# OrangeSodahub/ORV

Measured on AMD Instinct MI355X. Metric: denoise-steps/sec, higher is better.
Workload: dtype bf16; 1 GPU; configs[1]: CogVideoX-2B singleview 320x480x17f (latents [B,5,32,40,60], S=3226), DDIM 50-step schedule, guidance 1.0, trajectory-conditioned; batch_per_gpu=4, num_layers=30, parallelism=replica x1 (no collective), valid=True

## Files before the change

orv_amd/csrc/norm.hip:

```cpp
#include "common.hpp"
#include "mxfp8.hpp"

namespace {

#ifndef ORV_LN_WAVES
#define ORV_LN_WAVES 1
#endif
template <int CH, bool FULL, bool MX = false>
__global__ __launch_bounds__(256, ORV_LN_WAVES) void ln_mod_kernel(const bf16_t* __restrict__ x, long ldx, bf16_t* __restrict__ y,
                                                     long ldy, const bf16_t* __restrict__ gamma,
                                                     const bf16_t* __restrict__ beta, const float* __restrict__ scale,
                                                     const float* __restrict__ shift, long mod_b, long mod_g, int seq,
                                                     int n_text, int per_group, int rows, int D, float eps,
                                                     orv_rowmap_t xmap, uint8_t* __restrict__ mxs) {
    const int lane = threadIdx.x & 63;
    const int row = blockIdx.x * 4 + (threadIdx.x >> 6);
    if (row >= rows) return;
    const int nchunk = D >> 3;
    const long xrow = xmap.rows > 0 ? (long)(row / xmap.rows) * xmap.bstride + xmap.off + row % xmap.rows : row;
    const bf16_t* xr = x + xrow * ldx;
    uint4 raw[CH];
    int ce[CH];
    bool ok[CH];
#pragma unroll
// ... 175 lines not shown
#pragma unroll
        for (int k = 0; k < 16; ++k) o[vt_pos(k)] = vt_s[grp * 16 + k][d];
        bf16_t* dst = vT + ((long)(b * H + h) * 64 + d) * s_pad + s0 + grp * 16;
        uint4 a, c2;
        a.x = o[0] | ((uint32_t)o[1] << 16); a.y = o[2] | ((uint32_t)o[3] << 16);
        a.z = o[4] | ((uint32_t)o[5] << 16); a.w = o[6] | ((uint32_t)o[7] << 16);
        c2.x = o[8] | ((uint32_t)o[9] << 16); c2.y = o[10] | ((uint32_t)o[11] << 16);
        c2.z = o[12] | ((uint32_t)o[13] << 16); c2.w = o[14] | ((uint32_t)o[15] << 16);
        *(uint4*)dst = a;
        *(uint4*)(dst + 8) = c2;
    }
}

#ifndef ORV_LNR_WAVES
#define ORV_LNR_WAVES 3
#endif
__device__ __forceinline__ uint4 lnr_load(const bf16_t* p) {
#ifdef ORV_LNR_NT_LOAD
    typedef unsigned nt_u32x4 __attribute__((ext_vector_type(4)));
    const nt_u32x4 v = __builtin_nontemporal_load((const nt_u32x4*)p);
    return make_uint4(v[0], v[1], v[2], v[3]);
#else
    return *(const uint4*)p;
#endif
}
__device__ __forceinline__ void lnr_store(bf16_t* p, const uint4 u) {
#ifdef ORV_LNR_NT_STORE
    typedef unsigned nt_u32x4 __attribute__((ext_vector_type(4)));
    __builtin_nontemporal_store(nt_u32x4{u.x, u.y, u.z, u.w}, (nt_u32x4*)p);
#else
    *(uint4*)p = u;
#endif
}
template <int CH, bool PACKED = false, bool MX = false>
__global__ __launch_bounds__(256, ORV_LNR_WAVES) void ln_mod_rows_kernel(const bf16_t* __restrict__ x, long ldx, bf16_t* __restrict__ y, long ldy,
                                                             const bf16_t* __restrict__ gamma, const bf16_t* __restrict__ beta,
                                                             const float* __restrict__ scale, const float* __restrict__ shift, long mod_b,
                                                             long mod_g, int seq, int n_text, int per_group, int rows, int D, float eps, int R,
                                                             uint8_t* __restrict__ mxs) {
    const int lane = threadIdx.x & 63;
    const int w = blockIdx.x * 4 + (threadIdx.x >> 6);
    const int r0 = __builtin_amdgcn_readfirstlane(w * R);
    if (r0 >= rows) return;
    const int r1 = min(r0 + R, rows);
    const int nchunk = D >> 3;
    int ce[CH];
    bool ok[CH];
#pragma unroll
    for (int i = 0; i < CH; ++i) {
        const int c = lane + 64 * i;
        ok[i] = c < nchunk;
        ce[i] = min(c, nchunk - 1);
    }
    float gg[CH][8], hh[CH][8];
    long cur_off = -1;
    uint4 raw[CH];
#pragma unroll
    for (int i = 0; i < CH; ++i) raw[i] = lnr_load(x + (long)r0 * ldx + ce[i] * 8);
    for (int row = r0; row < r1; ++row) {
        const int b = row / seq, sidx = row % seq;
        const long off = b * mod_b + orv_group_of(sidx, n_text, per_group) * mod_g;
        if (off != cur_off) {
            cur_off = off;
#pragma unroll
            for (int i = 0; i < CH; ++i) {
                const uint4 gm = *(const uint4*)(gamma + ce[i] * 8), bt = *(const uint4*)(beta + ce[i] * 8);
                const float4 s0 = *(const float4*)(scale + off + ce[i] * 8), s1 = *(const float4*)(scale + off + ce[i] * 8 + 4);
                const float4 h0 = *(const float4*)(shift + off + ce[i] * 8), h1 = *(const float4*)(shift + off + ce[i] * 8 + 4);
                const float sv[8] = {s0.x, s0.y, s0.z, s0.w, s1.x, s1.y, s1.z, s1.w};
                const float hv[8] = {h0.x, h0.y, h0.z, h0.w, h1.x, h1.y, h1.z, h1.w};
                const uint32_t gw[4] = {gm.x, gm.y, gm.z, gm.w}, bw[4] = {bt.x, bt.y, bt.z, bt.w};
#pragma unroll
                for (int e = 0; e < 8; ++e) {
                    const float g = bf2f((e & 1) ? gw[e >> 1] >> 16 : gw[e >> 1] & 0xffff);
                    const float be = bf2f((e & 1) ? bw[e >> 1] >> 16 : bw[e >> 1] & 0xffff);
                    gg[i][e] = g * (1.0f + sv[e]);
                    hh[i][e] = fmaf(be, 1.0f + sv[e], hv[e]);
                }
                __builtin_amdgcn_sched_barrier(0);
            }
        }
        float v[CH][8];
        float s = 0.f;
#pragma unroll
        for (int i = 0; i < CH; ++i) {
            const uint32_t wv[4] = {raw[i].x, raw[i].y, raw[i].z, raw[i].w};
#pragma unroll
            for (int e = 0; e < 4; ++e) {
                v[i][2 * e] = bf2f(wv[e] & 0xffff);
                v[i][2 * e + 1] = bf2f(wv[e] >> 16);
                s += ok[i] ? v[i][2 * e] + v[i][2 * e + 1] : 0.f;
            }
        }
        {
            const int rn = min(row + 1, rows - 1);
#pragma unroll
            for (int i = 0; i < CH; ++i) raw[i] = lnr_load(x + (long)rn * ldx + ce[i] * 8);
        }
        const float mean = wave_sum_valu(s) / (float)D;
        float sq = 0.f;
#pragma unroll
        for (int i = 0; i < CH; ++i) {
#pragma unroll
            for (int e = 0; e < 8; ++e) {
                const float d = ok[i] ? v[i][e] - mean : 0.f;
                sq += d * d;
            }
        }
        const float rstd = rsqrtf(wave_sum_valu(sq) / (float)D + eps);
        bf16_t* yr = y + (long)row * ldy;
#pragma unroll
        for (int i = 0; i < CH; ++i) {
            float o[8];
#pragma unroll
            for (int e = 0; e < 8; ++e) o[e] = fmaf((v[i][e] - mean) * rstd, gg[i][e], hh[i][e]);
            uint4 u;
            u.x = pack2bf(o[0], o[1]); u.y = pack2bf(o[2], o[3]); u.z = pack2bf(o[4], o[5]); u.w = pack2bf(o[6], o[7]);
            if constexpr (MX) {
                uint2 qq;
                uint32_t sb;
                mx_quantize8(u, qq, sb);
                if (ok[i]) mx_store8((uint8_t*)y + (long)row * ldy, mxs + (long)row * (D >> 5), ce[i], qq, sb);
            } else if (PACKED) *(uint4*)(y + ((((long)(row >> 4) * (D >> 5) + (ce[i] >> 2)) << 9) + ((((ce[i] & 3) << 4) + (row & 15)) << 3))) = u;
            else lnr_store(yr + ce[i] * 8, u);
        }
    }
}

}

static int layernorm_modulate_impl(const void* x, int ldx, orv_rowmap_t xmap, void* y, int ldy, const void* gamma,
                                   const void* beta, const float* scale, const float* shift, long mod_b, long mod_g,
                                   orv_groups_t grp, int batch, int D, float eps, void* stream, bool packed, uint8_t* mxs = nullptr) {
    ORV_REQUIRE(x && y, "orv_layernorm_modulate: null operand");
    ORV_REQUIRE(D % 8 == 0 && D <= 4096, "orv_layernorm_modulate: D=%d must be a multiple of 8 and <= 4096", D);
    ORV_REQUIRE(grp.seq > 0 && batch > 0, "orv_layernorm_modulate: empty problem");
    ORV_REQUIRE((scale == nullptr) == (shift == nullptr), "orv_layernorm_modulate: scale and shift go together");
    ORV_REQUIRE(ldx % 8 == 0 && ldy % 8 == 0, "orv_layernorm_modulate: misaligned rows");
    const int rows = batch * grp.seq;
    const int ch = (D / 8 + 63) / 64;
    dim3 grid((rows + 3) / 4), block(256);
    hipStream_t st = (hipStream_t)stream;
    const bool full = gamma && beta && scale && shift;
    const bool mx = mxs != nullptr;
    ORV_REQUIRE(!mx || (!packed && D % 32 == 0), "orv_layernorm_modulate_mxfp8: D=%d must be a multiple of 32", D);
    static int rows_env = -2;
    if (rows_env == -2) { const char* e = getenv("ORV_LN_ROWS"); rows_env = e ? atoi(e) : -1; }
    ORV_REQUIRE(!packed || (full && xmap.rows == 0 && ch <= 4 && D % 32 == 0 && ldy == D),
                "orv_layernorm_modulate_packed: needs gamma, beta, scale, shift, no row map, D %% 32 == 0, D <= 2048 and ldy == D");
    if (full && xmap.rows == 0 && (packed || rows_env != 0) && ch <= 4) {
        const int slots = 256 * 4 * ORV_LNR_WAVES;
        const int R = rows_env > 0 ? rows_env : max(rows >= 2048 ? 2 : 1, (rows + slots - 1) / slots);
        dim3 g2(((rows + R - 1) / R + 3) / 4);
#define ORV_LNR_CASE(C)                                                                                                \
        if (mx)                                                                                                        \
            hipLaunchKernelGGL((ln_mod_rows_kernel<C, false, true>), g2, block, 0, st, (const bf16_t*)x, (long)ldx, (bf16_t*)y, (long)ldy, \
                               (const bf16_t*)gamma, (const bf16_t*)beta, scale, shift, mod_b, mod_g, grp.seq, grp.n_text, \
                               grp.per_group, rows, D, eps, R, mxs);                                                   \
        else if (packed)                                                                                               \
            hipLaunchKernelGGL((ln_mod_rows_kernel<C, true>), g2, block, 0, st, (const bf16_t*)x, (long)ldx, (bf16_t*)y, (long)ldy, \
                               (const bf16_t*)gamma, (const bf16_t*)beta, scale, shift, mod_b, mod_g, grp.seq, grp.n_text, \
                               grp.per_group, rows, D, eps, R, nullptr);                                               \
// ... 60 lines not shown
                            const float* rope_cos, const float* rope_sin, int B, int S, int H, int n_text, int s_pad,
                            float eps, float q_premul, void* stream) {
    return orv_qkv_prep_from(qkv, qkv, vT, gq, bq, gk, bk, rope_cos, rope_sin, B, S, H, n_text, s_pad, eps, q_premul, stream);
}

extern "C" int orv_qkv_prep_from(const void* src, void* qkv, void* vT, const void* gq, const void* bq, const void* gk,
                                 const void* bk, const float* rope_cos, const float* rope_sin, int B, int S, int H, int n_text,
                                 int s_pad, float eps, float q_premul, void* stream) {
    ORV_REQUIRE(src && qkv, "orv_qkv_prep: null operand");
    ORV_REQUIRE(B > 0 && S > 0 && H > 0, "orv_qkv_prep: empty problem");
    ORV_REQUIRE(s_pad % 64 == 0 && s_pad >= S && s_pad == ((S + 63) / 64) * 64,
                "orv_qkv_prep: s_pad=%d must be S=%d rounded up to 64", s_pad, S);
    ORV_REQUIRE((rope_cos == nullptr) == (rope_sin == nullptr), "orv_qkv_prep: cos and sin go together");
    dim3 grid(s_pad / 64, H, B);
    hipLaunchKernelGGL(qkv_prep_kernel, grid, dim3(256), 0, (hipStream_t)stream, (const bf16_t*)src, (bf16_t*)qkv, (bf16_t*)vT,
                       (const bf16_t*)gq, (const bf16_t*)bq, (const bf16_t*)gk, (const bf16_t*)bk, rope_cos, rope_sin, S,
                       H, n_text, s_pad, eps, q_premul);
    return orv_check_launch("orv_qkv_prep");
}

namespace {

struct ModArgs {
    const bf16_t* temb;
    const bf16_t* act;
    const bf16_t* const* W;
    const bf16_t* const* bias;
    float* out;
    int n_tab, B, T, E, width, text;
    int vis_tiles;
};

template <int KS>
__device__ __forceinline__ void mod_cond_frags(const ModArgs& p, int b, int t, bool is_text, bool rvalid, int hi, bf16x8 (&cf)[KS]) {
    const bool has_act = !is_text && p.act != nullptr;
    const bf16_t* tp = p.temb + (long)b * p.E + hi * 8;
    const bf16_t* ap = has_act ? p.act + ((long)b * p.T + t) * p.E + hi * 8 : tp;
    constexpr int BATCH = KS < 8 ? KS : 8;
#pragma unroll
    for (int k0 = 0; k0 < KS; k0 += BATCH) {
        uint4 tu[BATCH], au[BATCH];
#pragma unroll
        for (int j = 0; j < BATCH; ++j) { tu[j] = *(const uint4*)(tp + (k0 + j) * 16); au[j] = *(const uint4*)(ap + (k0 + j) * 16); }
#pragma unroll
        for (int j = 0; j < BATCH; ++j) {
            const uint32_t tw[4] = {tu[j].x, tu[j].y, tu[j].z, tu[j].w}, aw[4] = {au[j].x, au[j].y, au[j].z, au[j].w};
            union { bf16x8 v; uint32_t u[4]; } c;
#pragma unroll
            for (int e = 0; e < 4; ++e) {
                float lo = bf2f(tw[e] & 0xffff), hi2 = bf2f(tw[e] >> 16);
                const float lo_a = bf2f(f2bf(lo + bf2f(aw[e] & 0xffff))), hi_a = bf2f(f2bf(hi2 + bf2f(aw[e] >> 16)));
                lo = has_act ? lo_a : lo;
                hi2 = has_act ? hi_a : hi2;
                c.u[e] = rvalid ? pack2bf(silu(lo), silu(hi2)) : 0u;
            }
            cf[k0 + j] = c.v;
        }
    }
}

template <int KS>
__global__ __launch_bounds__(256) void mod_tables_kernel(const ModArgs p) {
    const int lane = threadIdx.x & 63, wave = threadIdx.x >> 6;
    const int l31 = lane & 31, hi = lane >> 5;
    const int tab = blockIdx.y;
    const bool is_text = (int)blockIdx.z >= p.vis_tiles;
    const int rtile = is_text ? blockIdx.z - p.vis_tiles : blockIdx.z;
    const int nrows = is_text ? p.B : p.B * p.T;
    const int r = rtile * 32 + l31;
    const bool rvalid = r < nrows;
// ... 30 lines not shown
                    o.x += bf2f(bb.x & 0xffff); o.y += bf2f(bb.x >> 16); o.z += bf2f(bb.y & 0xffff); o.w += bf2f(bb.y >> 16);
                }
                *(float4*)(orow + n) = o;
            }
        }
    }
}

}

namespace {
__device__ __forceinline__ void mt_glds16(const void* gsrc, const void* lds_dst) {
    unsigned keep;
    const unsigned d = __builtin_amdgcn_readfirstlane((unsigned)(uintptr_t)(const __attribute__((address_space(3))) char*)lds_dst);
    asm volatile("s_mov_b32 %0, m0\n\ts_mov_b32 m0, %2\n\ts_nop 0\n\tglobal_load_lds_dwordx4 %1, off\n\ts_mov_b32 m0, %0"
                 : "=&s"(keep) : "v"(gsrc), "s"(d) : "memory");
}
constexpr int MT_SLABS = 4;
constexpr int MT_MAXBLK = 4;
__global__ __launch_bounds__(256) void mod_tables_lds_kernel(const ModArgs p) {
    constexpr int KS = 32, SPB = 8;
    __shared__ __attribute__((aligned(16))) char smem[4 * MT_SLABS * 4096];
    const int lane = threadIdx.x & 63, wave = __builtin_amdgcn_readfirstlane(threadIdx.x >> 6);
    const int l31 = lane & 31, hi = lane >> 5, sw = (l31 >> 1) & 7;
    const int tab = blockIdx.y;
    const bool is_text = (int)blockIdx.z >= p.vis_tiles;
    const int rtile = is_text ? blockIdx.z - p.vis_tiles : blockIdx.z;
    const int nrows = is_text ? p.B : p.B * p.T;
    const int r = rtile * 32 + l31;
    const bool rvalid = r < nrows;
    const int b = rvalid ? (is_text ? r : r / p.T) : 0;
    const int t = rvalid && !is_text ? r % p.T : 0;
    bf16x8 cf[KS];
    mod_cond_frags<KS>(p, b, t, is_text, rvalid, hi, cf);
    const bf16_t* Wt = p.W[tab] + (is_text ? (long)p.width * p.E : 0);
    const bf16_t* bt = p.bias ? (p.bias[tab] ? p.bias[tab] + (is_text ? p.width : 0) : nullptr) : nullptr;
    const int G = 1 + p.T;
    float* orow = p.out + (((long)tab * p.B + b) * G + (is_text ? 0 : 1 + t)) * p.width;
    const int nblocks = p.width / 32;
    const int nb0 = blockIdx.x * 4 + wave, stride = gridDim.x * 4;
    const int nblk = nb0 < nblocks ? (nblocks - nb0 + stride - 1) / stride : 0;
    const int total = nblk * SPB;
    char* const ring = smem + wave * (MT_SLABS * 4096);
    int soff[4];
#pragma unroll
    for (int j = 0; j < 4; ++j) {
        const int row = 8 * j + (lane >> 3);
        soff[j] = row * p.E + (((lane & 7) ^ ((row >> 1) & 7)) << 3);
    }
    auto issue = [&](int sl) {
        const int bi = sl / SPB, ks = sl % SPB;
        const bf16_t* wp = Wt + (long)((nb0 + bi * stride) * 32) * p.E + ks * 64;
        char* const d = ring + (sl % MT_SLABS) * 4096;
#pragma unroll
        for (int j = 0; j < 4; ++j) mt_glds16(wp + soff[j], d + j * 1024);
    };
    f32x16 acc[MT_MAXBLK];
#pragma unroll
    for (int i = 0; i < MT_MAXBLK; ++i)
#pragma unroll
        for (int e = 0; e < 16; ++e) acc[i][e] = 0.f;
#pragma unroll
    for (int sl = 0; sl < MT_SLABS - 1; ++sl)
        if (sl < total) issue(sl);
    const int rd_off = l31 * 128;
#pragma unroll
    for (int bi = 0; bi < MT_MAXBLK; ++bi) {
// ... 70 lines not shown
```

orv_amd/csrc/gemm_d8.hip:

```cpp
#include "gemm_common.hpp"

namespace {
using namespace orv_gemm;

__device__ __forceinline__ void d8_unpack8(const uint4 u, float (&f)[8]) {
    f[0] = bf2f(u.x & 0xffff); f[1] = bf2f(u.x >> 16); f[2] = bf2f(u.y & 0xffff); f[3] = bf2f(u.y >> 16);
    f[4] = bf2f(u.z & 0xffff); f[5] = bf2f(u.z >> 16); f[6] = bf2f(u.w & 0xffff); f[7] = bf2f(u.w >> 16);
}
__device__ __forceinline__ uint4 d8_pack8(const float (&f)[8]) {
    return make_uint4(pack2bf(f[0], f[1]), pack2bf(f[2], f[3]), pack2bf(f[4], f[5]), pack2bf(f[6], f[7]));
}
__device__ __forceinline__ float d8_sum_quad(float v) {
    v += __uint_as_float(__builtin_amdgcn_update_dpp(0, __float_as_uint(v), 0xB1, 0xF, 0xF, true));
    v += __uint_as_float(__builtin_amdgcn_update_dpp(0, __float_as_uint(v), 0x4E, 0xF, 0xF, true));
    return v;
}
__device__ __forceinline__ float d8_shl4(float v) {
    return __uint_as_float(__builtin_amdgcn_update_dpp(0, __float_as_uint(v), 0x104, 0xF, 0xF, true));
}
__device__ __forceinline__ float d8_shr4(float v) {
    return __uint_as_float(__builtin_amdgcn_update_dpp(0, __float_as_uint(v), 0x114, 0xF, 0xF, true));
}
__device__ __forceinline__ unsigned long long d8_uniform64(unsigned long long u) {
    const unsigned lo = __builtin_amdgcn_readfirstlane((unsigned)u), hi = __builtin_amdgcn_readfirstlane((unsigned)(u >> 32));
    return ((unsigned long long)hi << 32) | lo;
}

#ifndef D8_RSETS
#define D8_RSETS 1
#endif
__device__ __forceinline__ void d8_glds_v(const void* gsrc, const char* lds_dst) {
    const unsigned d = __builtin_amdgcn_readfirstlane((unsigned)(uintptr_t)(const __attribute__((address_space(3))) char*)lds_dst);
    asm volatile("s_mov_b32 m0, %1\n\ts_nop 0\n\tglobal_load_lds_dwordx4 %0, off" :: "v"(gsrc), "s"(d) : "memory", "m0");
}
__device__ __forceinline__ void d8_issue_rows(const GemmArgs& p, const int row0, const int colg, const int lane, const char* slab) {
#pragma unroll
    for (int j = 0; j < 4; ++j) {
        const int mc = min(row0 + 8 * j + (lane >> 3), p.M - 1);
        long rr = mc;
        if (p.r_mod > 0) rr = mc % p.r_mod;
        else if (p.c_rows > 0) rr = (long)(mc / p.c_rows) * p.c_bstride + p.c_off + mc % p.c_rows;
        d8_glds_v(p.R + rr * p.ldr + colg + 8 * (lane & 7), slab + j * 1024);
    }
}
template <int BN, int EPI>
constexpr bool d8_rlds() {
#ifdef ORV_D8_RLDS
    return BN <= 192 && (EPI == 2 || EPI == 3);
#else
    return false;
#endif
}

template <int BN, int EPI, int RB = 2>
__device__ __forceinline__ void d8_epilogue(const GemmArgs& p, f32x4 (&acc)[RB][BN / 16], const int row0, const int col0, const int lane,
                                            char* const scr, const char* const rslab = nullptr) {
    constexpr int NG = BN / 64;
    constexpr bool RLDS = d8_rlds<BN, EPI>();
    const int g = lane >> 4, r16 = lane & 15;
    const int c = lane & 7, rr8 = lane >> 3;
    int woff[4];
#pragma unroll
    for (int blk = 0; blk < 4; ++blk) {
        const int L = 8 * (blk >> 1) + 2 * g + (blk & 1);
        woff[blk] = r16 * 256 + ((L ^ (r16 & 7)) << 4);
    }
    const int roff0 = rr8 * 256 + (((2 * c) ^ rr8) << 4), roff1 = rr8 * 256 + (((2 * c + 1) ^ rr8) << 4);

    long orow[RB][2];
    bool valid[RB][2];
#pragma unroll
    for (int rb = 0; rb < RB; ++rb)
#pragma unroll
        for (int j = 0; j < 2; ++j) {
            const int m = row0 + rb * 16 + 8 * j + rr8;
            valid[rb][j] = m < p.M;
            const int mc = min(m, p.M - 1);
            orow[rb][j] = mc;
            if (p.c_rows > 0) orow[rb][j] = (long)(mc / p.c_rows) * p.c_bstride + p.c_off + mc % p.c_rows;
        }
    const float* gate_row[2] = {nullptr, nullptr};
    bool gate_lane[2] = {false, false};
    if (EPI == 2 && p.gate) {
#pragma unroll
        for (int rb = 0; rb < RB; ++rb) {
            const int mf = __builtin_amdgcn_readfirstlane(row0 + rb * 16), ml = min(mf + 15, p.M - 1);
            long of = min(mf, p.M - 1), ol = ml;
            if (p.c_rows > 0) {
                of = (long)(of / p.c_rows) * p.c_bstride + p.c_off + of % p.c_rows;
                ol = (long)(ml / p.c_rows) * p.c_bstride + p.c_off + ml % p.c_rows;
            }
            const int bf_ = (int)(of / p.seq), bl_ = (int)(ol / p.seq);
            const int gf_ = orv_group_of((int)(of % p.seq), p.n_text, p.per_group);
            const int gl_ = orv_group_of((int)(ol % p.seq), p.n_text, p.per_group);
            if (bf_ == bl_ && gf_ == gl_) gate_row[rb] = p.gate + bf_ * p.gate_b + gf_ * p.gate_g;
            else gate_lane[rb] = true;
        }
    }
    constexpr int RS = (D8_RSETS == 0) ? (BN <= 192 ? NG : 1) : D8_RSETS;
    uint4 r8[RS][RB][2];
    auto load_rows = [&](int cg, uint4 (&dst)[RB][2]) {
        const int col8 = col0 + 64 * cg + 8 * c;
#pragma unroll
        for (int rb = 0; rb < RB; ++rb)
#pragma unroll
            for (int j = 0; j < 2; ++j) {
                const int mc = min(row0 + rb * 16 + 8 * j + rr8, p.M - 1);
                long rr = mc;
                if (p.r_mod > 0) rr = mc % p.r_mod;
                else if (p.c_rows > 0) rr = (long)(mc / p.c_rows) * p.c_bstride + p.c_off + mc % p.c_rows;
                dst[rb][j] = *(const uint4*)(p.R + rr * p.ldr + col8);
            }
    };
    auto take_rows = [&](int cg, uint4 (&dst)[RB][2]) {
        asm volatile("s_waitcnt vmcnt(0)" ::: "memory");
        __builtin_amdgcn_sched_barrier(0);
#pragma unroll
        for (int rb = 0; rb < RB; ++rb)
#pragma unroll
            for (int j = 0; j < 2; ++j) dst[rb][j] = *(const uint4*)(rslab + (rb * 16 + 8 * j + rr8) * 128 + c * 16);
        if (cg + 1 < NG) {
            asm volatile("s_waitcnt lgkmcnt(0)" ::: "memory");
            __builtin_amdgcn_sched_barrier(0);
            d8_issue_rows(p, row0, col0 + 64 * (cg + 1), lane, rslab);
        }
    };
    if (RLDS) {
        take_rows(0, r8[0]);
    } else if (EPI == 2 || EPI == 3) {
        load_rows(0, r8[0]);
        if (RS == NG && NG > 1 && !RLDS) {
#pragma unroll
            for (int cg = 1; cg < NG; ++cg) load_rows(cg, r8[cg % RS]);
        }
    }

#pragma unroll
    for (int cg = 0; cg < NG; ++cg) {
        const int col8 = col0 + 64 * cg + 8 * c;
        if (!RLDS && RS == 2 && RS != NG && (EPI == 2 || EPI == 3) && cg + 1 < NG) load_rows(cg + 1, r8[(cg + 1) & 1]);
        if (RLDS) { if (cg > 0) take_rows(cg, r8[0]); }
        else if (RS == 1 && (EPI == 2 || EPI == 3) && cg > 0) load_rows(cg, r8[0]);
        float b8[8];
#pragma unroll
        for (int e = 0; e < 8; ++e) b8[e] = 0.f;
        if (p.bias) d8_unpack8(*(const uint4*)(p.bias + col8), b8);
        float ga[8], be[8];
        int region = 2;
        float post = 1.f;
        if constexpr (EPI == 4) {
            region = __builtin_amdgcn_readfirstlane((col0 + 64 * cg) / (p.qn_heads * 64));
            const bf16_t* gam = region == 0 ? p.qn_gq : p.qn_gk;
            const bf16_t* bet = region == 0 ? p.qn_bq : p.qn_bk;
            post = region == 0 ? p.qn_premul : 1.f;
#pragma unroll
            for (int e = 0; e < 8; ++e) { ga[e] = 1.f; be[e] = 0.f; }
            if (region < 2 && gam) d8_unpack8(*(const uint4*)(gam + 8 * c), ga);
            if (region < 2 && bet) d8_unpack8(*(const uint4*)(bet + 8 * c), be);
        }
        float g8[8];
        const float* g_cached = nullptr;
#pragma unroll
        for (int e = 0; e < 8; ++e) g8[e] = 1.f;

#pragma unroll
        for (int rb = 0; rb < RB; ++rb) {
#pragma unroll
            for (int blk = 0; blk < 4; ++blk) *(f32x4*)(scr + woff[blk]) = acc[rb][4 * cg + blk];
            float v[2][8];
#pragma unroll
            for (int j = 0; j < 2; ++j) {
                const f32x4 lo = *(const f32x4*)(scr + j * 2048 + roff0), hi = *(const f32x4*)(scr + j * 2048 + roff1);
                v[j][0] = lo[0]; v[j][1] = lo[1]; v[j][2] = lo[2]; v[j][3] = lo[3];
                v[j][4] = hi[0]; v[j][5] = hi[1]; v[j][6] = hi[2]; v[j][7] = hi[3];
            }
            const bool g_lane = (EPI == 2 && p.gate) ? gate_lane[rb] : false;
            if (EPI == 2 && p.gate && !g_lane) {
                const float* gr = gate_row[rb];
                if (gr != g_cached) {
                    g_cached = gr;
                    const float4 a = *(const float4*)(gr + col8), b = *(const float4*)(gr + col8 + 4);
                    g8[0] = a.x; g8[1] = a.y; g8[2] = a.z; g8[3] = a.w; g8[4] = b.x; g8[5] = b.y; g8[6] = b.z; g8[7] = b.w;
                }
            }
#pragma unroll
            for (int j = 0; j < 2; ++j) {
                float (&w)[8] = v[j];
#pragma unroll
                for (int e = 0; e < 8; ++e) w[e] += b8[e];
                bf16_t* crow = p.C + orow[rb][j] * p.ldc + col8;
                if (p.Y && valid[rb][j]) *(uint4*)(p.Y + orow[rb][j] * p.ldy + col8) = d8_pack8(w);
                if constexpr (EPI == 4) {
                    if (region < 2) {
                        float hi[8];
#pragma unroll
                        for (int e = 0; e < 8; ++e) hi[e] = d8_shl4(w[e]);
                        float s = 0.f;
#pragma unroll
                        for (int e = 0; e < 8; ++e) s += w[e];
#pragma unroll
                        for (int e = 0; e < 8; ++e) s += hi[e];
                        s = d8_sum_quad(s);
                        const float s_up = d8_shr4(s);
                        const float mean = (c < 4 ? s : s_up) * (1.f / 64.f);
                        float sq = 0.f;
#pragma unroll
                        for (int e = 0; e < 8; ++e) { w[e] -= mean; sq = qkln_sq(w[e], sq); }
#pragma unroll
                        for (int e = 0; e < 8; ++e) { hi[e] -= mean; sq = qkln_sq(hi[e], sq); }
                        sq = d8_sum_quad(sq);
                        const float sq_up = d8_shr4(sq);
                        const float rstd = rsqrtf((c < 4 ? sq : sq_up) * (1.f / 64.f) + p.qn_eps);
#pragma unroll
                        for (int e = 0; e < 8; ++e) w[e] = qkln_affine(w[e], rstd, ga[e], be[e], post);
                    }
                }
                if (EPI == 1) {
#pragma unroll
                    for (int e = 0; e < 8; ++e) w[e] = gelu_tanh(w[e]);
                }
                if (EPI == 2) {
                    float rv[8], gg[8];
                    d8_unpack8(r8[RLDS ? 0 : cg % RS][rb][j], rv);
#pragma unroll
                    for (int e = 0; e < 8; ++e) gg[e] = g8[e];
                    if (g_lane) {
                        const int bidx = (int)(orow[rb][j] / p.seq), sq_ = (int)(orow[rb][j] % p.seq);
                        const float* grow = p.gate + bidx * p.gate_b + orv_group_of(sq_, p.n_text, p.per_group) * p.gate_g;
                        const float4 a = *(const float4*)(grow + col8), b = *(const float4*)(grow + col8 + 4);
                        gg[0] = a.x; gg[1] = a.y; gg[2] = a.z; gg[3] = a.w; gg[4] = b.x; gg[5] = b.y; gg[6] = b.z; gg[7] = b.w;
                    }
#pragma unroll
                    for (int e = 0; e < 8; ++e) w[e] = rv[e] + gg[e] * w[e];
                }
                if (EPI == 3) {
                    float rv[8];
                    d8_unpack8(r8[RLDS ? 0 : cg % RS][rb][j], rv);
#pragma unroll
                    for (int e = 0; e < 8; ++e) w[e] *= gelu_tanh_grad(rv[e]);
                }
                if (valid[rb][j]) *(uint4*)crow = d8_pack8(w);
            }
        }
    }
}

template <int BN, int EPI, int RB = 2>
__device__ __forceinline__ void d8_epilogue_packed(const GemmArgs& p, f32x4 (&acc)[RB][BN / 16], const int row0, const int col0, const int lane) {
    const int g = lane >> 4;
    const long nblk = p.ldc / 32;
#pragma unroll
    for (int P = 0; P < BN / 32; ++P) {
        float b8[8];
#pragma unroll
        for (int e = 0; e < 8; ++e) b8[e] = 0.f;
        if (p.bias) d8_unpack8(*(const uint4*)(p.bias + col0 + 32 * P + 8 * g), b8);
#pragma unroll
        for (int rb = 0; rb < RB; ++rb) {
            float v[8];
#pragma unroll
            for (int e = 0; e < 8; ++e) v[e] = acc[rb][2 * P + (e >> 2)][e & 3] + b8[e];
            if (EPI == 1) {
#pragma unroll
                for (int e = 0; e < 8; ++e) v[e] = gelu_tanh(v[e]);
            }
            char* blk = (char*)p.C + (((long)(row0 / 16 + rb) * nblk + (col0 / 32 + P)) << 10);
            *(uint4*)(blk + lane * 16) = d8_pack8(v);
        }
    }
}
// ... 187 lines not shown
        bufc = (bufc + 1) & 3;                                                                                       \
    }

    int bufc = 0;
    D8_ISSUE_W(0)
    D8_ISSUE_W(1) D8_ISSUE_A(a0)
    D8_ISSUE_W(2) D8_ISSUE_A(a1)
    asm volatile("s_waitcnt vmcnt(%0)" :: "n"(2 * (ND + NA)) : "memory");
    D8_FENCE() __builtin_amdgcn_s_barrier(); D8_FENCE()
    _Pragma("unroll") for (int s_ = 0; s_ < 2 * CBP; ++s_) { D8_READ1(s_ % CBP, s_ / CBP, 0, 0) }
    D8_FENCE()

    for (int tile = blockIdx.x; tile < ntiles; tile += gridDim.x) {
        D8_SETUP_W(wbn, tW + (int)gridDim.x)
        D8_SETUP_A(abn, tA + (int)gridDim.x)
        for (int kt = 0; kt < nk; kt += 3) {
            if (d8_rlds<BN, EPI>() && kt + 3 >= nk) {
                int tm_, tn_;
                tile_of_index(p, tile, ntiles, tm_, tn_);
                d8_issue_rows(p, tm_ * BM + wrb * 16, tn_ * BN, lane, smem + SCR + 8 * 4096 + wave * 4096);
            }
            D8_KTILE(a0, a2)
            D8_KTILE(a1, a0)
            D8_KTILE(a2, a1)
        }
        int tm, tn;
        tile_of_index(p, tile, ntiles, tm, tn);
#ifdef ORV_D8_ABL_NOEPI
        _Pragma("unroll") for (int a_ = 0; a_ < RB; ++a_)
            _Pragma("unroll") for (int b_ = 0; b_ < NCB; ++b_) asm volatile("" :: "v"(acc[a_][b_]));
#else
        if ((EPI == 0 || EPI == 1) && p.c_packed) d8_epilogue_packed<BN, EPI, RB>(p, acc, tm * BM + wrb * 16, tn * BN, lane);
        else d8_epilogue<BN, EPI, RB>(p, acc, tm * BM + wrb * 16, tn * BN, lane, smem + SCR + wave * 4096, smem + SCR + 8 * 4096 + wave * 4096);
#endif
#pragma unroll
        for (int a = 0; a < RB; ++a)
#pragma unroll
            for (int b = 0; b < NCB; ++b) acc[a][b] = f32x4{0.f, 0.f, 0.f, 0.f};
    }
    asm volatile("s_waitcnt vmcnt(0)" ::: "memory");
    asm volatile("" :: "v"(a0[0]), "v"(a1[0]), "v"(a2[0]), "v"(fx[0][0]));
}

template <int BN, int EPI>
__global__ __launch_bounds__(512) void gemm_d8_kernel(const GemmArgs p) {
    extern __shared__ __attribute__((aligned(16))) char smem[];
    d8_body<BN, EPI, 2, 256>(p, smem);
}
template <int BN, int EPI>
__global__ __launch_bounds__(512) void gemm_d8r192_kernel(const GemmArgs p) {
    extern __shared__ __attribute__((aligned(16))) char smem[];
    if (__builtin_amdgcn_readfirstlane(threadIdx.x >> 6) < 4) d8_body<BN, EPI, 2, 192>(p, smem);
    else d8_body<BN, EPI, 1, 192>(p, smem);
}

template <int BN, int EPI, int BM>
int launch_d8_one(const GemmArgs& a, hipStream_t st) {
    constexpr int smem = 4 * BN * 128 + 8 * 4096 + (d8_rlds<BN, EPI>() ? 8 * 4096 : 0);
    void (*kern)(const GemmArgs);
    if constexpr (BM == 256) kern = gemm_d8_kernel<BN, EPI>;
    else kern = gemm_d8r192_kernel<BN, EPI>;
    static bool attr_done = false;
    if (!attr_done) {
        (void)hipFuncSetAttribute((const void*)kern, hipFuncAttributeMaxDynamicSharedMemorySize, smem);
        attr_done = true;
    }
    int grid = min(a.tiles_m * a.tiles_n, orv_num_cus());
    if (a.grid_cap > 0) grid = min(grid, a.grid_cap);
    hipLaunchKernelGGL(kern, dim3(grid), dim3(512), smem, st, a);
    return orv_check_launch("orv_gemm_bf16");
}

}

namespace orv_gemm {
int launch_d8(const GemmArgs& a, int bn, int epi, hipStream_t st, int bm) {
    if (!a.a_packed || (long)a.N * a.ldw * 2 >= (1L << 32) || a.K % 192 != 0 || a.lda != a.K) {
        orv_set_error("orv_gemm_bf16: the d8 kernel needs a packed A (a_packed, lda == K), K %% 192 == 0 and W below 4 GiB (lda=%ld N=%d ldw=%ld K=%d)",
                      a.lda, a.N, a.ldw, a.K);
        return ORV_EINVAL;
    }
    if (a.c_packed && (epi > 1 || a.ldc != a.N || a.c_rows > 0 || a.Y)) {
        orv_set_error("orv_gemm_bf16: packed C needs epilogue 0 / 1, ldc == N, no row map, no Y");
        return ORV_EINVAL;
    }
    if (bm == 192) {
        if ((long)a.tiles_m * 192 > ((long)a.M + 255) / 256 * 256) {
            orv_set_error("orv_gemm_bf16: 192-row d8 tiles would read past the packed row slots (M=%d)", a.M);
            return ORV_EINVAL;
        }
        if (bn == 128) {
            switch (epi) {
                case 0: return launch_d8_one<128, 0, 192>(a, st);
                case 1: return launch_d8_one<128, 1, 192>(a, st);
                case 2: return launch_d8_one<128, 2, 192>(a, st);
                case 4: return launch_d8_one<128, 4, 192>(a, st);
            }
        } else if (bn == 192) {
            switch (epi) {
                case 0: return launch_d8_one<192, 0, 192>(a, st);
                case 1: return launch_d8_one<192, 1, 192>(a, st);
                case 2: return launch_d8_one<192, 2, 192>(a, st);
                case 4: return launch_d8_one<192, 4, 192>(a, st);
            }
        }
        orv_set_error("orv_gemm_bf16: no 192-row d8 kernel for BN=%d epilogue %d", bn, epi);
        return ORV_EINVAL;
    }
    if (bn == 256) {
        switch (epi) {
            case 0: return launch_d8_one<256, 0, 256>(a, st);
            case 1: return launch_d8_one<256, 1, 256>(a, st);
            case 2: return launch_d8_one<256, 2, 256>(a, st);
            case 3: return launch_d8_one<256, 3, 256>(a, st);
            case 4: return launch_d8_one<256, 4, 256>(a, st);
        }
    } else if (bn == 128) {
// ... 56 lines not shown
```

Baseline: 100.3 steps/s (clips x denoise steps per second).

## Share folded LN modulation factors via LDS and split cond-fragment loads across waves

In the row-wise LayerNorm-modulate kernel, the block cooperatively computes the folded gamma*(1+scale) and beta*(1+scale)+shift factors once for the block's first modulation group and stores them in shared memory. Waves whose rows share that group read these factors from LDS instead of each issuing redundant global loads and recomputing them. The trailing prefetch is also guarded so it no longer loads past the wave's row range, and an optional timestamp probe is added behind a macro. In the modulation-table kernel, each of the four waves now builds a quarter of the SiLU conditioning fragments and exchanges them through LDS, cutting redundant global reads at the cost of two block barriers.

```diff
diff --git a/orv_amd/csrc/norm.hip b/orv_amd/csrc/norm.hip
--- a/orv_amd/csrc/norm.hip
+++ b/orv_amd/csrc/norm.hip
@@ -231,16 +231,44 @@
     *(uint4*)p = u;
 #endif
 }
+__device__ __forceinline__ void lnr_fold(const bf16_t* __restrict__ gamma, const bf16_t* __restrict__ beta, const float* __restrict__ scale,
+                                         const float* __restrict__ shift, long off, int c, float (&g)[8], float (&h)[8]) {
+    const uint4 gm = *(const uint4*)(gamma + c * 8), bt = *(const uint4*)(beta + c * 8);
+    const float4 s0 = *(const float4*)(scale + off + c * 8), s1 = *(const float4*)(scale + off + c * 8 + 4);
+    const float4 h0 = *(const float4*)(shift + off + c * 8), h1 = *(const float4*)(shift + off + c * 8 + 4);
+    const float sv[8] = {s0.x, s0.y, s0.z, s0.w, s1.x, s1.y, s1.z, s1.w};
+    const float hv[8] = {h0.x, h0.y, h0.z, h0.w, h1.x, h1.y, h1.z, h1.w};
+    const uint32_t gw[4] = {gm.x, gm.y, gm.z, gm.w}, bw[4] = {bt.x, bt.y, bt.z, bt.w};
+#pragma unroll
+    for (int e = 0; e < 8; ++e) {
+        const float ga = bf2f((e & 1) ? gw[e >> 1] >> 16 : gw[e >> 1] & 0xffff);
+        const float be = bf2f((e & 1) ? bw[e >> 1] >> 16 : bw[e >> 1] & 0xffff);
+        g[e] = ga * (1.0f + sv[e]);
+        h[e] = fmaf(be, 1.0f + sv[e], hv[e]);
+    }
+}
+#ifdef ORV_LNR_STAMP
+constexpr int LNR_STAMP_WAVES = 8192;
+__device__ unsigned long long lnr_stamp[3 * LNR_STAMP_WAVES];
+__device__ __forceinline__ void lnr_stamp_put(unsigned long long t0, unsigned long long t1, unsigned long long t2) {
+    const int w = blockIdx.x * 4 + (threadIdx.x >> 6);
+    if ((threadIdx.x & 63) == 0 && w < LNR_STAMP_WAVES) { lnr_stamp[3 * w] = t0; lnr_stamp[3 * w + 1] = t1; lnr_stamp[3 * w + 2] = t2; }
+}
+#endif
 template <int CH, bool PACKED = false, bool MX = false>
 __global__ __launch_bounds__(256, ORV_LNR_WAVES) void ln_mod_rows_kernel(const bf16_t* __restrict__ x, long ldx, bf16_t* __restrict__ y, long ldy,
                                                              const bf16_t* __restrict__ gamma, const bf16_t* __restrict__ beta,
                                                              const float* __restrict__ scale, const float* __restrict__ shift, long mod_b,
                                                              long mod_g, int seq, int n_text, int per_group, int rows, int D, float eps, int R,
                                                              uint8_t* __restrict__ mxs) {
+    __shared__ float4 fac[4][CH * 64];
+#ifdef ORV_LNR_STAMP
+    const unsigned long long st0 = __builtin_amdgcn_s_memrealtime();
+    unsigned long long st1 = st0;
+#endif
     const int lane = threadIdx.x & 63;
     const int w = blockIdx.x * 4 + (threadIdx.x >> 6);
     const int r0 = __builtin_amdgcn_readfirstlane(w * R);
-    if (r0 >= rows) return;
     const int r1 = min(r0 + R, rows);
     const int nchunk = D >> 3;
     int ce[CH];
@@ -251,32 +279,46 @@
         ok[i] = c < nchunk;
         ce[i] = min(c, nchunk - 1);
     }
+    auto mod_off = [&](int row) { return (row / seq) * mod_b + orv_group_of(row % seq, n_text, per_group) * mod_g; };
+    auto load_row = [&](uint4 (&raw)[CH], int row) {
+#pragma unroll
+        for (int i = 0; i < CH; ++i) raw[i] = lnr_load(x + (long)row * ldx + ce[i] * 8);
+    };
+    uint4 raw[CH];
+    if (r0 < r1) load_row(raw, r0);
+    const long off0 = mod_off(blockIdx.x * 4 * R);
+    if (CH == 4 || threadIdx.x < CH * 64) {
+        float g[8], h[8];
+        lnr_fold(gamma, beta, scale, shift, off0, min((int)threadIdx.x, nchunk - 1), g, h);
+        fac[0][threadIdx.x] = make_float4(g[0], g[1], g[2], g[3]);
+        fac[1][threadIdx.x] = make_float4(g[4], g[5], g[6], g[7]);
+        fac[2][threadIdx.x] = make_float4(h[0], h[1], h[2], h[3]);
+        fac[3][threadIdx.x] = make_float4(h[4], h[5], h[6], h[7]);
+    }
+    __syncthreads();
     float gg[CH][8], hh[CH][8];
     long cur_off = -1;
-    uint4 raw[CH];
-#pragma unroll
-    for (int i = 0; i < CH; ++i) raw[i] = lnr_load(x + (long)r0 * ldx + ce[i] * 8);
     for (int row = r0; row < r1; ++row) {
-        const int b = row / seq, sidx = row % seq;
-        const long off = b * mod_b + orv_group_of(sidx, n_text, per_group) * mod_g;
+        const long off = mod_off(row);
         if (off != cur_off) {
             cur_off = off;
-#pragma unroll
-            for (int i = 0; i < CH; ++i) {
-                const uint4 gm = *(const uint4*)(gamma + ce[i] * 8), bt = *(const uint4*)(beta + ce[i] * 8);
-                const float4 s0 = *(const float4*)(scale + off + ce[i] * 8), s1 = *(const float4*)(scale + off + ce[i] * 8 + 4);
-                const float4 h0 = *(const float4*)(shift + off + ce[i] * 8), h1 = *(const float4*)(shift + off + ce[i] * 8 + 4);
-                const float sv[8] = {s0.x, s0.y, s0.z, s0.w, s1.x, s1.y, s1.z, s1.w};
-                const float hv[8] = {h0.x, h0.y, h0.z, h0.w, h1.x, h1.y, h1.z, h1.w};
-                const uint32_t gw[4] = {gm.x, gm.y, gm.z, gm.w}, bw[4] = {bt.x, bt.y, bt.z, bt.w};
-#pragma unroll
-                for (int e = 0; e < 8; ++e) {
-                    const float g = bf2f((e & 1) ? gw[e >> 1] >> 16 : gw[e >> 1] & 0xffff);
-                    const float be = bf2f((e & 1) ? bw[e >> 1] >> 16 : bw[e >> 1] & 0xffff);
-                    gg[i][e] = g * (1.0f + sv[e]);
-                    hh[i][e] = fmaf(be, 1.0f + sv[e], hv[e]);
+            if (off == off0) {
+#pragma unroll
+                for (int i = 0; i < CH; ++i) {
+                    const float4 g0 = fac[0][ce[i]], g1 = fac[1][ce[i]], h0 = fac[2][ce[i]], h1 = fac[3][ce[i]];
+                    gg[i][0] = g0.x; gg[i][1] = g0.y; gg[i][2] = g0.z; gg[i][3] = g0.w;
+                    gg[i][4] = g1.x; gg[i][5] = g1.y; gg[i][6] = g1.z; gg[i][7] = g1.w;
+                    hh[i][0] = h0.x; hh[i][1] = h0.y; hh[i][2] = h0.z; hh[i][3] = h0.w;
+                    hh[i][4] = h1.x; hh[i][5] = h1.y; hh[i][6] = h1.z; hh[i][7] = h1.w;
                 }
-                __builtin_amdgcn_sched_barrier(0);
+            } else {
+#pragma unroll
+                for (int i = 0; i < CH; ++i) {
+                    int c = ce[i];
+                    asm volatile("" : "+v"(c));
+                    lnr_fold(gamma, beta, scale, shift, off, c, gg[i], hh[i]);
+                    __builtin_amdgcn_sched_barrier(0);
+                }
             }
         }
         float v[CH][8];
@@ -291,11 +333,7 @@
                 s += ok[i] ? v[i][2 * e] + v[i][2 * e + 1] : 0.f;
             }
         }
-        {
-            const int rn = min(row + 1, rows - 1);
-#pragma unroll
-            for (int i = 0; i < CH; ++i) raw[i] = lnr_load(x + (long)rn * ldx + ce[i] * 8);
-        }
+        if (row + 1 < r1) load_row(raw, row + 1);
         const float mean = wave_sum_valu(s) / (float)D;
         float sq = 0.f;
 #pragma unroll
@@ -323,10 +361,26 @@
             } else if (PACKED) *(uint4*)(y + ((((long)(row >> 4) * (D >> 5) + (ce[i] >> 2)) << 9) + ((((ce[i] & 3) << 4) + (row & 15)) << 3))) = u;
             else lnr_store(yr + ce[i] * 8, u);
         }
-    }
-}
-
-}
+#ifdef ORV_LNR_STAMP
+        if (row == r0) { __builtin_amdgcn_sched_barrier(0); st1 = __builtin_amdgcn_s_memrealtime(); __builtin_amdgcn_sched_barrier(0); }
+#endif
+    }
+#ifdef ORV_LNR_STAMP
+    if (r0 < r1) lnr_stamp_put(st0, st1, __builtin_amdgcn_s_memrealtime());
+#endif
+}
+
+}
+
+#ifdef ORV_LNR_STAMP
+extern "C" int orv_lnr_stamp_read(unsigned long long* out) {
+    if (hipDeviceSynchronize() != hipSuccess) return ORV_EINVAL;
+    if (out && hipMemcpyFromSymbol(out, HIP_SYMBOL(lnr_stamp), sizeof(unsigned long long) * 3 * LNR_STAMP_WAVES) != hipSuccess) return ORV_EINVAL;
+    void* p = nullptr;
+    if (hipGetSymbolAddress(&p, HIP_SYMBOL(lnr_stamp)) != hipSuccess) return ORV_EINVAL;
+    return hipMemset(p, 0, sizeof(unsigned long long) * 3 * LNR_STAMP_WAVES) == hipSuccess ? 0 : ORV_EINVAL;
+}
+#endif
 
 static int layernorm_modulate_impl(const void* x, int ldx, orv_rowmap_t xmap, void* y, int ldy, const void* gamma,
                                    const void* beta, const float* scale, const float* shift, long mod_b, long mod_g,
@@ -453,10 +507,10 @@
 };
 
 template <int KS>
-__device__ __forceinline__ void mod_cond_frags(const ModArgs& p, int b, int t, bool is_text, bool rvalid, int hi, bf16x8 (&cf)[KS]) {
+__device__ __forceinline__ void mod_cond_frags(const ModArgs& p, int b, int t, bool is_text, bool rvalid, int hi, bf16x8 (&cf)[KS], int k_first = 0) {
     const bool has_act = !is_text && p.act != nullptr;
-    const bf16_t* tp = p.temb + (long)b * p.E + hi * 8;
-    const bf16_t* ap = has_act ? p.act + ((long)b * p.T + t) * p.E + hi * 8 : tp;
+    const bf16_t* tp = p.temb + (long)b * p.E + hi * 8 + k_first * 16;
+    const bf16_t* ap = has_act ? p.act + ((long)b * p.T + t) * p.E + hi * 8 + k_first * 16 : tp;
     constexpr int BATCH = KS < 8 ? KS : 8;
 #pragma unroll
     for (int k0 = 0; k0 < KS; k0 += BATCH) {
@@ -553,7 +607,17 @@
     const int b = rvalid ? (is_text ? r : r / p.T) : 0;
     const int t = rvalid && !is_text ? r % p.T : 0;
     bf16x8 cf[KS];
-    mod_cond_frags<KS>(p, b, t, is_text, rvalid, hi, cf);
+    {
+        bf16x8 part[KS / 4];
+        mod_cond_frags<KS / 4>(p, b, t, is_text, rvalid, hi, part, wave * (KS / 4));
+        bf16x8* const stage = (bf16x8*)smem;
+#pragma unroll
+        for (int j = 0; j < KS / 4; ++j) stage[(wave * (KS / 4) + j) * 64 + lane] = part[j];
+        __syncthreads();
+#pragma unroll
+        for (int k = 0; k < KS; ++k) cf[k] = stage[k * 64 + lane];
+        __syncthreads();
+    }
     const bf16_t* Wt = p.W[tab] + (is_text ? (long)p.width * p.E : 0);
     const bf16_t* bt = p.bias ? (p.bias[tab] ? p.bias[tab] + (is_text ? p.width : 0) : nullptr) : nullptr;
     const int G = 1 + p.T;
```

After: 101.0 steps/s (clips x denoise steps per second), median of 6. About the same (+0.6%).

## Rework d8 residual/gate epilogue: per-lane bias/gate loads spread via bpermute, streaming residual prefetch

Applied to the files above, without the earlier changes.

Rewrites the residual and gated-residual epilogues of the d8 GEMM. Bias and gate vectors are now loaded once per column group as one value per lane and spread to lanes with ds_bpermute, replacing repeated 8-wide vector loads. The gate lookup is classified per wave into one segment, two segments, or per-row, and residual rows are prefetched one column group ahead per row instead of through register sets. Row indices shrink to 32-bit for BN=256 to save registers, at the cost of a new launch check on row count and seq. For BN=256 it also adds an extra LDS read/fence sequence after the epilogue.

```diff
diff --git a/orv_amd/csrc/gemm_d8.hip b/orv_amd/csrc/gemm_d8.hip
--- a/orv_amd/csrc/gemm_d8.hip
+++ b/orv_amd/csrc/gemm_d8.hip
@@ -1,4 +1,5 @@
 #include "gemm_common.hpp"
+#include <type_traits>
 
 namespace {
 using namespace orv_gemm;
@@ -26,9 +27,6 @@
     return ((unsigned long long)hi << 32) | lo;
 }
 
-#ifndef D8_RSETS
-#define D8_RSETS 1
-#endif
 __device__ __forceinline__ void d8_glds_v(const void* gsrc, const char* lds_dst) {
     const unsigned d = __builtin_amdgcn_readfirstlane((unsigned)(uintptr_t)(const __attribute__((address_space(3))) char*)lds_dst);
     asm volatile("s_mov_b32 m0, %1\n\ts_nop 0\n\tglobal_load_lds_dwordx4 %0, off" :: "v"(gsrc), "s"(d) : "memory", "m0");
@@ -67,7 +65,9 @@
     }
     const int roff0 = rr8 * 256 + (((2 * c) ^ rr8) << 4), roff1 = rr8 * 256 + (((2 * c + 1) ^ rr8) << 4);
 
-    long orow[RB][2];
+    constexpr bool GATH = EPI == 2 || EPI == 3;
+    using row_t = std::conditional_t<GATH && BN == 256, int, long>;
+    row_t orow[RB][2];
     bool valid[RB][2];
 #pragma unroll
     for (int rb = 0; rb < RB; ++rb)
@@ -77,40 +77,46 @@
             valid[rb][j] = m < p.M;
             const int mc = min(m, p.M - 1);
             orow[rb][j] = mc;
-            if (p.c_rows > 0) orow[rb][j] = (long)(mc / p.c_rows) * p.c_bstride + p.c_off + mc % p.c_rows;
-        }
-    const float* gate_row[2] = {nullptr, nullptr};
-    bool gate_lane[2] = {false, false};
+            if (p.c_rows > 0) orow[rb][j] = (row_t)((long)(mc / p.c_rows) * p.c_bstride + p.c_off + mc % p.c_rows);
+        }
+    const float *gate_a = nullptr, *gate_b = nullptr;
+    int gseg = 0;
+    bool in_a[RB][2];
+#pragma unroll
+    for (int rb = 0; rb < RB; ++rb) in_a[rb][0] = in_a[rb][1] = true;
     if (EPI == 2 && p.gate) {
-#pragma unroll
-        for (int rb = 0; rb < RB; ++rb) {
-            const int mf = __builtin_amdgcn_readfirstlane(row0 + rb * 16), ml = min(mf + 15, p.M - 1);
-            long of = min(mf, p.M - 1), ol = ml;
-            if (p.c_rows > 0) {
-                of = (long)(of / p.c_rows) * p.c_bstride + p.c_off + of % p.c_rows;
-                ol = (long)(ml / p.c_rows) * p.c_bstride + p.c_off + ml % p.c_rows;
-            }
-            const int bf_ = (int)(of / p.seq), bl_ = (int)(ol / p.seq);
-            const int gf_ = orv_group_of((int)(of % p.seq), p.n_text, p.per_group);
-            const int gl_ = orv_group_of((int)(ol % p.seq), p.n_text, p.per_group);
-            if (bf_ == bl_ && gf_ == gl_) gate_row[rb] = p.gate + bf_ * p.gate_b + gf_ * p.gate_g;
-            else gate_lane[rb] = true;
-        }
-    }
-    constexpr int RS = (D8_RSETS == 0) ? (BN <= 192 ? NG : 1) : D8_RSETS;
-    uint4 r8[RS][RB][2];
-    auto load_rows = [&](int cg, uint4 (&dst)[RB][2]) {
-        const int col8 = col0 + 64 * cg + 8 * c;
-#pragma unroll
-        for (int rb = 0; rb < RB; ++rb)
-#pragma unroll
-            for (int j = 0; j < 2; ++j) {
-                const int mc = min(row0 + rb * 16 + 8 * j + rr8, p.M - 1);
-                long rr = mc;
-                if (p.r_mod > 0) rr = mc % p.r_mod;
-                else if (p.c_rows > 0) rr = (long)(mc / p.c_rows) * p.c_bstride + p.c_off + mc % p.c_rows;
-                dst[rb][j] = *(const uint4*)(p.R + rr * p.ldr + col8);
-            }
+        const int mf = __builtin_amdgcn_readfirstlane(row0);
+        long of = min(mf, p.M - 1), ol = min(mf + 16 * RB - 1, p.M - 1);
+        if (p.c_rows > 0) {
+            of = (long)(of / p.c_rows) * p.c_bstride + p.c_off + of % p.c_rows;
+            ol = (long)(ol / p.c_rows) * p.c_bstride + p.c_off + ol % p.c_rows;
+        }
+        const int bf_ = (int)(of / p.seq), bl_ = (int)(ol / p.seq);
+        const int gf_ = orv_group_of((int)(of % p.seq), p.n_text, p.per_group);
+        const int gl_ = orv_group_of((int)(ol % p.seq), p.n_text, p.per_group);
+        gate_a = p.gate + bf_ * p.gate_b + gf_ * p.gate_g;
+        gseg = 1;
+        if (bf_ != bl_ || gf_ != gl_) {
+            gate_b = p.gate + bl_ * p.gate_b + gl_ * p.gate_g;
+            const int ea_ = gf_ == 0 ? p.n_text : (p.per_group > 0 ? p.n_text + gf_ * p.per_group : p.seq);
+            const long end_a = (long)bf_ * p.seq + min(ea_, p.seq);
+            const long start_b = (long)bl_ * p.seq + (gl_ == 0 ? 0 : p.n_text + (gl_ - 1) * max(p.per_group, 0));
+            bool other = false;
+#pragma unroll
+            for (int rb = 0; rb < RB; ++rb)
+#pragma unroll
+                for (int j = 0; j < 2; ++j) {
+                    in_a[rb][j] = orow[rb][j] < end_a;
+                    other = other || !(in_a[rb][j] || orow[rb][j] >= start_b);
+                }
+            gseg = (BN == 256 || __builtin_amdgcn_ballot_w64(other) != 0) ? 3 : 2;
+        }
+    }
+    uint4 r8[RB][2];
+    auto load_row = [&](int cg, int rb, int j) {
+        long rr = orow[rb][j];
+        if (p.r_mod > 0) rr = min(row0 + rb * 16 + 8 * j + rr8, p.M - 1) % p.r_mod;
+        return *(const uint4*)(p.R + rr * p.ldr + col0 + 64 * cg + 8 * c);
     };
     auto take_rows = [&](int cg, uint4 (&dst)[RB][2]) {
         asm volatile("s_waitcnt vmcnt(0)" ::: "memory");
@@ -126,25 +132,57 @@
         }
     };
     if (RLDS) {
-        take_rows(0, r8[0]);
-    } else if (EPI == 2 || EPI == 3) {
-        load_rows(0, r8[0]);
-        if (RS == NG && NG > 1 && !RLDS) {
-#pragma unroll
-            for (int cg = 1; cg < NG; ++cg) load_rows(cg, r8[cg % RS]);
-        }
-    }
+        take_rows(0, r8);
+    } else if (GATH) {
+#pragma unroll
+        for (int rb = 0; rb < RB; ++rb)
+#pragma unroll
+            for (int j = 0; j < 2; ++j) r8[rb][j] = load_row(0, rb, j);
+    }
+    const int bp = c << 5;
+    uint32_t bsrc[NG];
+    float gsrc_a[NG], gsrc_b[NG];
+#pragma unroll
+    for (int cg = 0; cg < NG; ++cg) { bsrc[cg] = 0; gsrc_a[cg] = gsrc_b[cg] = 1.f; }
+    if constexpr (GATH) {
+        if (p.bias) {
+#pragma unroll
+            for (int cg = 0; cg < NG; ++cg) bsrc[cg] = p.bias[col0 + 64 * cg + lane];
+        }
+        if (gseg == 1 || gseg == 2) {
+#pragma unroll
+            for (int cg = 0; cg < NG; ++cg) gsrc_a[cg] = gate_a[col0 + 64 * cg + lane];
+        }
+        if (gseg == 2) {
+#pragma unroll
+            for (int cg = 0; cg < NG; ++cg) gsrc_b[cg] = gate_b[col0 + 64 * cg + lane];
+        }
+    }
+    auto spread8 = [&](uint32_t src, uint32_t (&o)[8]) {
+        asm volatile("ds_bpermute_b32 %0, %8, %9\n\tds_bpermute_b32 %1, %8, %9 offset:4\n\tds_bpermute_b32 %2, %8, %9 offset:8\n\t"
+                     "ds_bpermute_b32 %3, %8, %9 offset:12\n\tds_bpermute_b32 %4, %8, %9 offset:16\n\tds_bpermute_b32 %5, %8, %9 offset:20\n\t"
+                     "ds_bpermute_b32 %6, %8, %9 offset:24\n\tds_bpermute_b32 %7, %8, %9 offset:28\n\ts_waitcnt lgkmcnt(0)"
+                     : "=&v"(o[0]), "=&v"(o[1]), "=&v"(o[2]), "=&v"(o[3]), "=&v"(o[4]), "=&v"(o[5]), "=&v"(o[6]), "=&v"(o[7])
+                     : "v"(bp), "v"(src));
+    };
 
 #pragma unroll
     for (int cg = 0; cg < NG; ++cg) {
         const int col8 = col0 + 64 * cg + 8 * c;
-        if (!RLDS && RS == 2 && RS != NG && (EPI == 2 || EPI == 3) && cg + 1 < NG) load_rows(cg + 1, r8[(cg + 1) & 1]);
-        if (RLDS) { if (cg > 0) take_rows(cg, r8[0]); }
-        else if (RS == 1 && (EPI == 2 || EPI == 3) && cg > 0) load_rows(cg, r8[0]);
+        if (RLDS && cg > 0) take_rows(cg, r8);
         float b8[8];
 #pragma unroll
         for (int e = 0; e < 8; ++e) b8[e] = 0.f;
-        if (p.bias) d8_unpack8(*(const uint4*)(p.bias + col8), b8);
+        if (p.bias) {
+            if constexpr (GATH) {
+                uint32_t o[8];
+                spread8(bsrc[cg], o);
+#pragma unroll
+                for (int e = 0; e < 8; ++e) b8[e] = bf2f((bf16_t)o[e]);
+            } else {
+                d8_unpack8(*(const uint4*)(p.bias + col8), b8);
+            }
+        }
         float ga[8], be[8];
         int region = 2;
         float post = 1.f;
@@ -159,33 +197,38 @@
             if (region < 2 && bet) d8_unpack8(*(const uint4*)(bet + 8 * c), be);
         }
         float g8[8];
-        const float* g_cached = nullptr;
 #pragma unroll
         for (int e = 0; e < 8; ++e) g8[e] = 1.f;
+        if (gseg == 1 || gseg == 2) {
+            uint32_t o[8];
+            spread8(__float_as_uint(gsrc_a[cg]), o);
+#pragma unroll
+            for (int e = 0; e < 8; ++e) g8[e] = __uint_as_float(o[e]);
+        }
 
 #pragma unroll
         for (int rb = 0; rb < RB; ++rb) {
 #pragma unroll
             for (int blk = 0; blk < 4; ++blk) *(f32x4*)(scr + woff[blk]) = acc[rb][4 * cg + blk];
             float v[2][8];
-#pragma unroll
-            for (int j = 0; j < 2; ++j) {
+            auto read_v = [&](int j) {
                 const f32x4 lo = *(const f32x4*)(scr + j * 2048 + roff0), hi = *(const f32x4*)(scr + j * 2048 + roff1);
                 v[j][0] = lo[0]; v[j][1] = lo[1]; v[j][2] = lo[2]; v[j][3] = lo[3];
                 v[j][4] = hi[0]; v[j][5] = hi[1]; v[j][6] = hi[2]; v[j][7] = hi[3];
-            }
-            const bool g_lane = (EPI == 2 && p.gate) ? gate_lane[rb] : false;
-            if (EPI == 2 && p.gate && !g_lane) {
-                const float* gr = gate_row[rb];
-                if (gr != g_cached) {
-                    g_cached = gr;
-                    const float4 a = *(const float4*)(gr + col8), b = *(const float4*)(gr + col8 + 4);
-                    g8[0] = a.x; g8[1] = a.y; g8[2] = a.z; g8[3] = a.w; g8[4] = b.x; g8[5] = b.y; g8[6] = b.z; g8[7] = b.w;
+            };
+            if constexpr (!GATH) { read_v(0); read_v(1); }
+#pragma unroll
+            for (int j = 0; j < 2; ++j) {
+                if constexpr (GATH) {
+                    asm volatile("" ::: "memory");
+                    read_v(j);
                 }
-            }
-#pragma unroll
-            for (int j = 0; j < 2; ++j) {
                 float (&w)[8] = v[j];
+                uint4 rcur;
+                if constexpr (GATH) {
+                    rcur = r8[rb][j];
+                    if (!RLDS && cg + 1 < NG) r8[rb][j] = load_row(cg + 1, rb, j);
+                }
 #pragma unroll
                 for (int e = 0; e < 8; ++e) w[e] += b8[e];
                 bf16_t* crow = p.C + orow[rb][j] * p.ldc + col8;
@@ -221,21 +264,35 @@
                 }
                 if (EPI == 2) {
                     float rv[8], gg[8];
-                    d8_unpack8(r8[RLDS ? 0 : cg % RS][rb][j], rv);
+                    d8_unpack8(rcur, rv);
 #pragma unroll
                     for (int e = 0; e < 8; ++e) gg[e] = g8[e];
-                    if (g_lane) {
-                        const int bidx = (int)(orow[rb][j] / p.seq), sq_ = (int)(orow[rb][j] % p.seq);
-                        const float* grow = p.gate + bidx * p.gate_b + orv_group_of(sq_, p.n_text, p.per_group) * p.gate_g;
-                        const float4 a = *(const float4*)(grow + col8), b = *(const float4*)(grow + col8 + 4);
-                        gg[0] = a.x; gg[1] = a.y; gg[2] = a.z; gg[3] = a.w; gg[4] = b.x; gg[5] = b.y; gg[6] = b.z; gg[7] = b.w;
+                    if (gseg == 2) {
+                        uint32_t o[8];
+                        spread8(__float_as_uint(gsrc_b[cg]), o);
+#pragma unroll
+                        for (int e = 0; e < 8; ++e) gg[e] = in_a[rb][j] ? g8[e] : __uint_as_float(o[e]);
+                    }
+                    if (gseg == 3 && j == 0) {
+                        f32x4 q[2][2];
+#pragma unroll
+                        for (int jj = 0; jj < 2; ++jj) {
+                            const unsigned o_ = (unsigned)orow[rb][jj];
+                            const int bidx = (int)(o_ / (unsigned)p.seq), sq_ = (int)(o_ - (unsigned)bidx * (unsigned)p.seq);
+                            const float* grow = p.gate + bidx * p.gate_b + orv_group_of(sq_, p.n_text, p.per_group) * p.gate_g;
+                            q[jj][0] = *(const f32x4*)(grow + col8);
+                            q[jj][1] = *(const f32x4*)(grow + col8 + 4);
+                        }
+                        asm volatile("" : "+v"(q[0][0]), "+v"(q[0][1]), "+v"(q[1][0]), "+v"(q[1][1]));
+#pragma unroll
+                        for (int e = 0; e < 8; ++e) { gg[e] = q[0][e >> 2][e & 3]; g8[e] = q[1][e >> 2][e & 3]; }
                     }
 #pragma unroll
                     for (int e = 0; e < 8; ++e) w[e] = rv[e] + gg[e] * w[e];
                 }
                 if (EPI == 3) {
                     float rv[8];
-                    d8_unpack8(r8[RLDS ? 0 : cg % RS][rb][j], rv);
+                    d8_unpack8(rcur, rv);
 #pragma unroll
                     for (int e = 0; e < 8; ++e) w[e] *= gelu_tanh_grad(rv[e]);
                 }
@@ -489,6 +546,11 @@
 #else
         if ((EPI == 0 || EPI == 1) && p.c_packed) d8_epilogue_packed<BN, EPI, RB>(p, acc, tm * BM + wrb * 16, tn * BN, lane);
         else d8_epilogue<BN, EPI, RB>(p, acc, tm * BM + wrb * 16, tn * BN, lane, smem + SCR + wave * 4096, smem + SCR + 8 * 4096 + wave * 4096);
+        if constexpr (BN == 256 && (EPI == 2 || EPI == 3)) {
+            D8_FENCE()
+            _Pragma("unroll") for (int s_ = 0; s_ < 2 * CBP; ++s_) { D8_READ1(s_ % CBP, s_ / CBP, bufc * BUFSZ, 0) }
+            D8_FENCE()
+        }
 #endif
 #pragma unroll
         for (int a = 0; a < RB; ++a)
@@ -540,6 +602,13 @@
     if (a.c_packed && (epi > 1 || a.ldc != a.N || a.c_rows > 0 || a.Y)) {
         orv_set_error("orv_gemm_bf16: packed C needs epilogue 0 / 1, ldc == N, no row map, no Y");
         return ORV_EINVAL;
+    }
+    if (epi == 2 || epi == 3) {
+        const long last = a.c_rows > 0 ? (long)((a.M - 1) / a.c_rows) * a.c_bstride + a.c_off + a.c_rows - 1 : (long)a.M - 1;
+        if (last >= (1L << 31) || (epi == 2 && a.gate && a.seq <= 0)) {
+            orv_set_error("orv_gemm_bf16: the row-operand epilogues need output rows below 2^31 and seq > 0 (last row %ld, seq=%d)", last, a.seq);
+            return ORV_EINVAL;
+        }
     }
     if (bm == 192) {
         if ((long)a.tiles_m * 192 > ((long)a.M + 255) / 256 * 256) {
```

New measurement: 102.9 steps/s (clips x denoise steps per second) before, 103.9 steps/s (clips x denoise steps per second) after (median of 6 runs). +1.1%, better.
